# mackelab/poisson-gpfa

Hardware: AMD Instinct MI355X
Metric: EM iterations/sec (higher is better)
Workload: dtype f64

## Files before the change

poisson-gpfa_amd/csrc/core.hip:

```cpp
#include "ctx.h"
#include "model.h"
#include "dual.h"

using namespace pgpfa;

thread_local std::string g_err;
thread_local unsigned long long g_fail_count = 0;

int fail(const char* fmt, ...) {
  char buf[1024];
  va_list ap;
  va_start(ap, fmt);
  vsnprintf(buf, sizeof(buf), fmt, ap);
  va_end(ap);
  g_err = buf;
  ++g_fail_count;
  return 1;
}

int ensure_hbuf(pgpfa_ctx* c, size_t len) {
  if (len <= c->hbuf_len) return 0;
  if (c->hbuf) hipHostFree(c->hbuf);
  c->hbuf = nullptr;
  HIPC(hipHostMalloc((void**)&c->hbuf, len * sizeof(double)));
// ... 606 lines not shown
    hipLaunchKernelGGL((rbf_pivchol2_kernel<256, 4>), dim3(p), dim3(1024), pivchol2_lds(T, rmax, 1024, 4), st, c->Flr, Tp, T, c->tau, c->bin, c->eps, c->lr_tol, rmax,
                       c->d_rank);
  else if (T > 256)
    hipLaunchKernelGGL((rbf_pivchol_kernel<512, 2>), dim3(p), dim3(1024), shm, st, c->Flr, Tp, T, c->tau, c->bin, c->eps, c->lr_tol, rmax, c->d_rank);
  else
    hipLaunchKernelGGL((rbf_pivchol_kernel<256, 1>), dim3(p), dim3(256), shm, st, c->Flr, Tp, T, c->tau, c->bin, c->eps, c->lr_tol, rmax, c->d_rank);
  HIPC(hipGetLastError());
  return 0;
}

int build_lowrank(pgpfa_ctx* c, bool pivchol_launched) {
  const int p = c->p, T = c->T, Tp = c->Tp;
  if (pivchol_launched) HIPC(hipStreamWaitEvent(c->st, c->ev_join, 0));
  else CHK(launch_pivchol(c, c->st));
  std::vector<int> r(p);
  CHK(dl_enqueue(c, r.data(), c->d_rank, sizeof(int) * p));
  CHK(dl_flush(c));
  const bool thin_all = c->thin_products >= 2 && c->mfma && T >= 4;
  const int G = ((c->rank_gran == 4 || c->rank_gran == 8) && thin_all) ? c->rank_gran : 16;
  c->rk.assign(p, 0);
  c->roff.assign(p + 1, 0);
  c->rr.assign(p, 0);
  c->roff16.assign(p + 1, 0);
  int extent = 0;
  for (int k = 0; k < p; ++k) {
    c->rr[k] = round_up(std::max(r[k], 1), G);
    c->rk[k] = round_up(c->rr[k], 16);
    c->roff[k + 1] = c->roff[k] + c->rr[k];
    c->roff16[k + 1] = c->roff16[k] + c->rk[k];
    extent = std::max(extent, c->roff[k] + c->rk[k]);
  }
  c->rtot = c->roff[p];
  c->rtot16 = c->roff16[p];
  c->rank_compact = (G != 16);
  c->rpad = round_up(std::max(c->rtot, extent), NB);
  const int nblk = round_up(c->rtot16, NB) / 16;
  std::vector<int> lat(nblk, -1), col(nblk, 0);
  for (int k = 0; k < p; ++k)
    for (int b = c->roff16[k] / 16; b < c->roff16[k + 1] / 16; ++b) { lat[b] = k; col[b] = b * 16 - c->roff16[k]; }
  CHK(upload_list(c, c->d_blk_lat, lat));
  CHK(upload_list(c, c->d_blk_col, col));
  CHK(upload_list(c, c->d_roff, c->roff));
  CHK(upload_list(c, c->d_roff16, c->roff16));
  if (c->rank_compact) {
    const int n16 = round_up(c->rtot16, NB);
    std::vector<int> cmap(n16, -1), pmap(round_up(c->rtot, 16) + 16, 0);
    for (int k = 0; k < p; ++k)
      for (int j = 0; j < c->rr[k]; ++j) { cmap[c->roff16[k] + j] = c->roff[k] + j; pmap[c->roff[k] + j] = c->roff16[k] + j; }
    std::vector<int> nrtab((round_up(c->rtot, 16)) / 16, 0);
    for (size_t b = 0; b < nrtab.size(); ++b) {
      const int last = std::min((int)b * 16 + 15, c->rtot - 1);
      nrtab[b] = std::min(c->rtot16, round_up(pmap[last] + 1, 16));
    }
    CHK(upload_list(c, c->d_cmap, cmap));
    CHK(upload_list(c, c->d_nrtab, nrtab));
  }
  {
    std::vector<int> tft, tf;
    c->kr_ft_len = 0; c->kr_f_len = 0;
    for (int k = 0; k < p; ++k) {
      const int kb = (k * T) / 16 * 16, ke = std::min(c->npad, round_up((k + 1) * T, 16));
      for (int r0 = c->roff[k]; r0 < c->roff[k + 1]; r0 += 64) { tft.push_back(r0); tft.push_back(c->roff[k + 1]); tft.push_back(kb); tft.push_back(ke); }
      c->kr_ft_len = std::max(c->kr_ft_len, ke - kb);
      for (int i0 = k * T; i0 < (k + 1) * T; i0 += 64) { tf.push_back(i0); tf.push_back((k + 1) * T); tf.push_back(c->roff[k]); tf.push_back(c->roff[k + 1]); }
      c->kr_f_len = std::max(c->kr_f_len, c->rk[k]);
    }
    c->ntab_ft = (int)tft.size() / 4; c->ntab_f = (int)tf.size() / 4;
    if (tft.size() > c->tab_cap || tf.size() > c->tab_cap) return fail("internal: row-tile table overflow");
    CHK(upload_list(c, c->d_kr_ft, tft));
    CHK(upload_list(c, c->d_kr_f, tf));
    std::vector<int> hft, hf;
    for (int k = 0; k < p; ++k) {
      const int ngr = (c->rr[k] + 63) / 64, per = round_up((c->rr[k] + ngr - 1) / ngr, 4);
      for (int m0 = 0; m0 < c->rr[k]; m0 += per) { hft.push_back(k); hft.push_back(m0); hft.push_back(std::min(per, c->rr[k] - m0)); hft.push_back(c->roff[k]); }
      for (int t0 = 0; t0 < T; t0 += 256) { hf.push_back(k); hf.push_back(t0); hf.push_back(c->rk[k]); hf.push_back(c->roff[k]); }
    }
    std::vector<int> hs;
    for (int m0 = 0; m0 < c->rtot; m0 += 64) { hs.push_back(0); hs.push_back(m0); hs.push_back(std::min(64, c->rtot - m0)); hs.push_back(0); }
    c->nthin_s = (int)hs.size() / 4;
    if (hs.size() > c->tab_cap) return fail("internal: thin-product table overflow");
    CHK(upload_list(c, c->d_thin_s, hs));
    c->nthin_ft = (int)hft.size() / 4; c->nthin_f = (int)hf.size() / 4;
    if (hft.size() > c->tab_cap || hf.size() > c->tab_cap) return fail("internal: thin-product table overflow");
    CHK(upload_list(c, c->d_thin_ft, hft));
    CHK(upload_list(c, c->d_thin_f, hf));
  }
  if ((size_t)c->rpad <= (size_t)c->ld) {
    HIPC(hipMemsetAsync(c->Fbig, 0, (size_t)c->ld * c->rpad * sizeof(double), c->st));
    HIPC(hipMemsetAsync(c->FTbig, 0, (size_t)c->rpad * c->ld * sizeof(double), c->st));
    int rkmax = 0;
    for (int k = 0; k < p; ++k) rkmax = std::max(rkmax, c->rk[k]);
    hipLaunchKernelGGL(build_fbig_kernel, dim3(rkmax, p), dim3(128), 0, c->st, c->Flr, Tp, T, c->d_roff, c->Fbig, c->ld, c->FTbig, c->rpad);
    HIPC(hipGetLastError());
  }
  c->info["lowrank_rtot"] = c->rtot;
  c->info["lowrank_rtot16"] = c->rtot16;
  c->info["lowrank_compact"] = c->rank_compact ? 1.0 : 0.0;
  c->flr32_valid = false;
  return 0;
}


int resolve_trials(pgpfa_ctx* c, int n, const int32_t* idx, Trials* out, bool distinct) {
  if (idx == nullptr) {
    out->v.resize(c->R);
    for (int i = 0; i < c->R; ++i) out->v[i] = i;
// ... 35 lines not shown
  int ndev = 0;
  hipError_t e = hipGetDeviceCount(&ndev);
  if (e != hipSuccess || ndev < 1) return fail("no HIP device available (%s)", hipGetErrorString(e));
  if (device < 0 || device >= ndev) return fail("device %d out of range (%d devices)", device, ndev);
  HIPC(hipSetDevice(device));
  pgpfa_ctx* c = new pgpfa_ctx();
  c->device = device; c->q = q; c->p = p; c->T = T; c->R = R; c->bin = bin_ms;
  c->n = p * T;
  c->npad = round_up(c->n, NB);
  c->ld = c->npad;
  c->Tp = round_up(T, NB);
  hipError_t se = hipStreamCreateWithFlags(&c->st, hipStreamNonBlocking);
  if (se != hipSuccess) { delete c; return fail("hipStreamCreate: %s", hipGetErrorString(se)); }
  if (hipStreamCreateWithFlags(&c->st2, hipStreamNonBlocking) != hipSuccess || hipEventCreateWithFlags(&c->ev_fork, hipEventDisableTiming) != hipSuccess ||
      hipEventCreateWithFlags(&c->ev_join, hipEventDisableTiming) != hipSuccess) {
    (void)hipGetLastError();
    if (c->st2) { hipStreamDestroy(c->st2); c->st2 = nullptr; }
  }
  int rc = 0;
  const size_t slab = (size_t)c->Tp * c->Tp;
  rc |= dmalloc(c, &c->Y, (size_t)R * q * T);
  rc |= dmalloc(c, &c->C, (size_t)q * p); rc |= dmalloc(c, &c->d, q); rc |= dmalloc(c, &c->tau, p);
  rc |= dmalloc(c, &c->Kpad, slab * p); rc |= dmalloc(c, &c->Kinv, slab * p);
  rc |= dmalloc(c, &c->Xmode, (size_t)R * c->n + 64, true);
  rc |= dmalloc(c, &c->Xprev, (size_t)R * c->n + 64, true);
  c->mode_serial.assign(R, -10); c->prev_serial.assign(R, -10);
  rc |= dmalloc(c, &c->vsm, (size_t)R * T * p * p + 2048, true);
  rc |= dmalloc(c, &c->Pauto, slab * p, true);
  rc |= dmalloc(c, &c->Pacc, slab * p, true);
  c->gemm_part_len = (size_t)16 << 20;
  rc |= dmalloc(c, &c->gemm_part, c->gemm_part_len);
  c->qpad = round_up(q, 16);
  c->ccu_cols = round_up(p * (p + 1) / 2, 16);
  if (p <= 16) {
    dispatch_pw(p, [&](auto pw) { constexpr int PW = decltype(pw)::value; c->ccu_cols = round_up(PW * (PW + 1) / 2, 16); });
    rc |= dmalloc(c, &c->CCu, (size_t)c->qpad * c->ccu_cols + 64, true);
    rc |= dmalloc(c, &c->C16, (size_t)c->qpad * 16 + 64, true);
  }
  c->dual_npd = round_up(p * (p + 1) / 2, 16);
  c->dual_ncol = c->dual_npd + round_up(p, 16);
  rc |= dmalloc(c, &c->dual_tbl, (size_t)round_up(q, 128) * c->dual_ncol + 4096, true);
  rc |= dmalloc(c, &c->ppart, (size_t)p * (PACC_SPLITS + 1) * T * T + 256);
  c->vsmgp_ok.assign(R, 0);
  c->trial_snap.assign(R, -1);
  c->trial_dual.assign(R, 0);
  c->lam_resident.assign(R, 0);
  c->lam_valid.assign(R, 0);
  rc |= dmalloc(c, &c->Flr, slab * p + 256 * (size_t)c->Tp, true);
  rc |= dmalloc(c, &c->d_rank, p); rc |= dmalloc(c, &c->d_roff, p + 1); rc |= dmalloc(c, &c->d_roff16, p + 1);
  rc |= dmalloc(c, &c->d_cmap, (size_t)p * c->Tp + 2 * NB + 64); rc |= dmalloc(c, &c->d_nrtab, (size_t)p * c->Tp / 16 + 64);
  c->tab_cap = 4 * ((size_t)c->ld / 64 + 2 * (size_t)p + 4);
  rc |= dmalloc(c, &c->d_kr_ft, c->tab_cap); rc |= dmalloc(c, &c->d_kr_f, c->tab_cap);
  rc |= dmalloc(c, &c->sink, 128, true);
  rc |= dmalloc(c, &c->d_thin_ft, c->tab_cap); rc |= dmalloc(c, &c->d_thin_f, c->tab_cap); rc |= dmalloc(c, &c->d_thin_s, c->tab_cap);
  rc |= dmalloc(c, &c->Fbig, (size_t)c->ld * c->ld + 256 * (size_t)c->ld, true); rc |= dmalloc(c, &c->FTbig, (size_t)c->ld * c->ld + 256 * (size_t)c->ld, true);
  rc |= dmalloc(c, &c->Gbar, (size_t)T * p * p + 64); rc |= dmalloc(c, &c->Wtbar, (size_t)T * p * p + 64); rc |= dmalloc(c, &c->d_blk_lat, (size_t)p * c->Tp / 16 + 64); rc |= dmalloc(c, &c->d_blk_col, (size_t)p * c->Tp / 16 + 64);
  rc |= dmalloc(c, &c->vec, (size_t)q * (p + 1));
  rc |= dmalloc(c, &c->cdpart, (size_t)1024 * (p + 2) * q);
  rc |= dmalloc(c, &c->cdout, (size_t)(p + 2) * q + 8);
  rc |= dmalloc(c, &c->cdym, (size_t)(p + 1) * q + 8);
  rc |= dmalloc(c, &c->cdym_part, (size_t)1024 * (p + 1) * q);
  rc |= dmalloc(c, &c->last_trials, R);
  {
    const size_t NH = 1 + (size_t)(p + 1) + (size_t)(p + 1) * (p + 2) / 2;
    rc |= dmalloc(c, &c->cdhpart, (size_t)128 * NH * q);
    rc |= dmalloc(c, &c->cdhout, NH * q + 8);
    rc |= dmalloc(c, &c->cdcenter, (size_t)q * (p + 1));
    rc |= dmalloc(c, &c->cdpack, (size_t)q * (p + 3) + 8);
  }
  if (hipHostMalloc((void**)&c->h_pcg, 4 * sizeof(int), hipHostMallocMapped) != hipSuccess ||
      hipHostGetDevicePointer((void**)&c->d_hpcg, c->h_pcg, 0) != hipSuccess) { (void)hipGetLastError(); c->h_pcg = nullptr; c->d_hpcg = nullptr; }
  rc |= alloc_cholws(c, &c->kws, p * TAU_MULTI_MAX, c->Tp, true);
  c->kws.nact = round_up(T, 64);
  {
    const size_t nqmax = (size_t)p * TAU_MULTI_MAX;
    rc |= dmalloc(c, &c->tK, slab * nqmax); rc |= dmalloc(c, &c->tM, slab * nqmax); rc |= dmalloc(c, &c->tA1, slab * nqmax);
    rc |= dmalloc(c, &c->tA2, slab * nqmax);
    rc |= dmalloc(c, &c->tscal, 16 + 8 * nqmax); rc |= dmalloc(c, &c->tpart, 1024 + 64 * nqmax);
  }
  if (rc) { pgpfa_destroy(c); return 1; }
  e = hipStreamSynchronize(c->st);
  if (e != hipSuccess) { pgpfa_destroy(c); return fail("sync: %s", hipGetErrorString(e)); }
  if (const char* g = std::getenv("PGPFA_RANK_GRAN")) { const int v = std::atoi(g); if (v == 4 || v == 8 || v == 16) c->rank_gran = v; }
  c->info["n_pad"] = c->npad;
  c->info["counts_two_bytes"] = 0.0;
  c->info["arena_bytes"] = 0.0;
  c->info["last_eps_wt_norm"] = 0.0;
  c->info["last_eps_wt_rms"] = 0.0;
  c->info["last_split_cov"] = 0.0;
  c->info["last_yt_mix_fused"] = 0.0;
  for (const char* k : {"plan_ms_total", "plans", "set_params_calls", "last_retry_ms", "last_dense_retries", "last_param_step", "last_param_step_prev",
                        "last_fallback_no_descent", "last_fallback_line_search", "last_fallback_outer_cap", "arena_grow_ms_total", "last_cold_restarts"}) c->info[k] = 0.0;
  *out = c;
  return 0;
}

int pgpfa_destroy(pgpfa_ctx* c) {
  if (!c) return 0;
  hipSetDevice(c->device);
  if (c->st) hipStreamSynchronize(c->st);
  if (c->comm) ncclCommDestroy(c->comm);
  for (void* p : c->allocs) hipFree(p);
  if (c->vsmgp) hipFree(c->vsmgp);
  if (c->Flr32) hipFree(c->Flr32);
  if (c->lam_keep) hipFree(c->lam_keep);
  if (c->split_buf) hipFree(c->split_buf);
  if (c->Yhi) hipFree(c->Yhi);
  arena_release(c);
  if (c->hbuf) hipHostFree(c->hbuf);
  if (c->dl_stage) hipHostFree(c->dl_stage);
  if (c->hibuf) hipHostFree(c->hibuf);
  if (c->ring) hipHostFree(c->ring);
  if (c->h_pcg) hipHostFree(c->h_pcg);
  if (c->h_seq) hipHostFree(c->h_seq);
  for (auto e : c->prof.pool) hipEventDestroy(e);
  if (c->st2) { hipStreamSynchronize(c->st2); hipStreamDestroy(c->st2); }
  if (c->tau_pin) hipHostFree(c->tau_pin);
  if (c->ev_tau_fork) hipEventDestroy(c->ev_tau_fork);
  if (c->ev_tau_done) hipEventDestroy(c->ev_tau_done);
  if (c->ev_fork) hipEventDestroy(c->ev_fork);
  if (c->ev_join) hipEventDestroy(c->ev_join);
  if (c->st) hipStreamDestroy(c->st);
  delete c;
  return 0;
}

int pgpfa_set_option(pgpfa_ctx* c, const char* key, double v) {
  if (!c || !key) return fail("null argument");
  const std::string k(key);
  if (k == "newton_xtol") c->xtol = v;
  else if (k == "newton_max_iter") c->max_iter = (int)v;
  else if (k == "use_mfma") {
    const bool was = c->mfma;
    c->mfma = (v != 0.0);
    if (c->have_params && c->rank_gran != 16 && was != c->mfma)
      CHK(pgpfa_set_params(c, std::vector<double>(c->hC).data(), std::vector<double>(c->hd).data(), std::vector<double>(c->htau).data()));
  }
  else if (k == "cd_mfma") c->cd_mfma = (v != 0.0);
  else if (k == "cd_hess_mfma") c->cd_hess_mfma = (v != 0.0);
  else if (k == "cross_kernel") c->cross_kernel = (v != 0.0);
  else if (k == "cd_debug") c->cd_debug = (int)v;
  else if (k == "pcg_fused") c->pcg_fused = (int)v;
  else if (k == "pcg_w32") c->pcg_w32 = (v != 0.0);
  else if (k == "pcg_form") c->pcg_form = (int)v;
  else if (k == "pcg_vec32") c->pcg_vec32 = (int)v;
  else if (k == "pcg_rx32") c->pcg_rx32 = (int)v;
  else if (k == "pcg_adapt") c->pcg_adapt = (int)v;
  else if (k == "pcg_xcd") c->pcg_xcd = (int)v;
  else if (k == "mt_fill") c->mt_fill = (int)v;
  else if (k == "overlap_factors") c->overlap_factors = (int)v;
  else if (k == "mix_slot") c->mix_slot = (int)v;
  else if (k == "yt_mix") c->yt_mix = (v != 0.0);
  else if (k == "pivchol_pairs") c->pivchol_pairs = (v != 0.0);
  else if (k == "vsm_b4") c->vsm_b4 = (int)v;
  else if (k == "poisson_tiles") c->poisson_tiles = (int)v;
  else if (k == "yt_mix_dbg") c->yt_mix_dbg = (int)v;
  else if (k == "syrk_dbg") c->syrk_dbg = (int)v;
  else if (k == "syrk_tile") c->syrk_tile = (int)v;
  else if (k == "mix_wide") c->mix_wide = (int)v;
  else if (k == "thin_products") {
    const bool was = c->thin_products >= 2;
    c->thin_products = (int)v;
    if (c->have_params && c->rank_gran != 16 && was != (c->thin_products >= 2))
      CHK(pgpfa_set_params(c, std::vector<double>(c->hC).data(), std::vector<double>(c->hd).data(), std::vector<double>(c->htau).data()));
  }
  else if (k == "copy_kernels") c->copy_kernels = (v != 0.0);
  else if (k == "chord") c->chord = (v != 0.0);
  else if (k == "shared_pcg") c->shared_pcg = (v != 0.0);
  else if (k == "time_newton") c->time_newton = (v != 0.0);
  else if (k == "pcg_trace") c->pcg_trace = (v != 0.0);
  else if (k == "measure_mix") { c->measure_mix = (v != 0.0); c->info["last_eps_wt_norm"] = 0.0; c->info["last_eps_wt_rms"] = 0.0; }
  else if (k == "pcg_retire") c->pcg_retire = (v != 0.0);
  else if (k == "split_cov") c->split_cov = (v != 0.0);
  else if (k == "split_max_norm") c->split_max_norm = v;
  else if (k == "cov_mode") c->cov_mode = (int)v;
  else if (k == "lowrank_tol") {
    const bool changed = c->lr_tol != v;
    c->lr_tol = v;
    if (c->have_params && changed)
      CHK(pgpfa_set_params(c, std::vector<double>(c->hC).data(), std::vector<double>(c->hd).data(), std::vector<double>(c->htau).data()));
  }
  else if (k == "keep_trial_vsmgp") c->keep_trial_vsmgp = (v != 0.0);
  else if (k == "dual_lowrank") c->dual_lowrank = (v != 0.0);
  else if (k == "dual_f32") c->dual_f32 = (int)v;
  else if (k == "slab_row_align") c->slab_row_align = (v != 0.0);
  else if (k == "vsm_mfma") c->vsm_mfma = (v != 0.0);
  else if (k == "dual_gemm") c->dual_gemm = (v != 0.0);
  else if (k == "extrapolate_start") c->extrapolate = (v != 0.0);
  else if (k == "extrapolate_beta") c->extrapolate_beta = v;
  else if (k == "extrapolate_guard") c->extrapolate_guard = v;
  else if (k == "start_guard") c->start_guard = (v != 0.0);
  else if (k == "shared_min") c->shared_min = (int)v;
  else if (k == "pcg_inner") c->pcg_inner_max = std::max(1, (int)v);
  else if (k == "pcg_eta0") c->pcg_eta0 = v;
  else if (k == "splitk_target") c->splitk_target = std::max(1, (int)v);
  else if (k == "small_tile_below") c->small_tile_below = (int)v;
  else if (k == "f32_tile64") c->f32_tile64 = (int)v;
  else if (k == "splitk_below64") c->splitk_below64 = (int)v;
  else if (k == "pcg_outer_max") c->pcg_outer_max = (int)v;
  else if (k == "chord_xtol") c->chord_xtol = v;
  else if (k == "chord_rho") c->chord_rho = v;
  else if (k == "chord_max_step") c->chord_max_step = v;
  else if (k == "chord_max") c->chord_max = (int)v;
  else if (k == "chunk_trials") { if (c->B > 0) return fail("chunk_trials must be set before the first E-step"); c->chunk_opt = (int)v; }
  else if (k == "workspace_headroom") c->arena_headroom = std::max(1.0, v);
  else if (k == "rank_gran") { if (v != 4.0 && v != 8.0 && v != 16.0) return fail("rank_gran is 4, 8 or 16"); c->rank_gran = (int)v; if (c->have_params) CHK(pgpfa_set_params(c, std::vector<double>(c->hC).data(), std::vector<double>(c->hd).data(), std::vector<double>(c->htau).data())); }
  else if (k == "workspace_pool") { if (c->arena_cap > 0) return fail("workspace_pool must be set before the first E-step"); c->use_pool = (v != 0.0); }
  else if (k == "workspace_grow_budget_ms") c->grow_budget_ms = v;
  else if (k == "workspace_grow_floor_slots") c->grow_floor_slots = std::max(1, (int)v);
// ... 312 lines not shown
```

poisson-gpfa_amd/csrc/cov.hip:

```cpp
#include "ctx.h"
#include "model.h"
#include "split.h"
#include "ytmix.h"

using namespace pgpfa;

template <typename TIN>
void launch_post_vsm(pgpfa_ctx* c, const TIN* Mt, long long sM, int ncol, int ns, int full_range, const int* roff = nullptr, int ts = 0) {
  const int T = c->T, p = c->p;
  if (ts <= 0) ts = T;
  if (p > 10 && c->vsm_mfma) {
    const int CB = post_vsm_mfma_cb(p, sizeof(TIN) == 4);
    if (p <= 20 && c->vsm_b4) {
      constexpr int VW = 16 / (int)sizeof(TIN);
      const bool vec = c->vsm_b4 >= 2 && T % VW == 0 && ts % VW == 0 && c->ld % VW == 0 && sM % VW == 0 && (((size_t)Mt) & 15) == 0;
      auto go = [&](auto nbk, auto vv) {
        constexpr int NBK = decltype(nbk)::value;
        constexpr bool VEC = decltype(vv)::value;
        const size_t lds4 = (size_t)CB * post_vsm_b4_cs(p, VEC) * sizeof(TIN);
        constexpr int BINS = VEC ? 64 : 32;
        (void)hipFuncSetAttribute(reinterpret_cast<const void*>(&post_vsm_b4_kernel<NBK, TIN, VEC>), hipFuncAttributeMaxDynamicSharedMemorySize, (int)lds4);
        hipLaunchKernelGGL((post_vsm_b4_kernel<NBK, TIN, VEC>), dim3((T + BINS - 1) / BINS, ns), dim3(512), lds4, c->st, Mt, sM, c->ld, ncol, T, p, c->vsm,
                           c->ident, c->trial_of_slot, full_range, CB, roff, (int)GBN, ts);
      };
// ... 74 lines not shown
      g.M = T; g.N = T; g.K = c->npad - kal; g.alpha = 1.0; g.beta = 0.0;
      g.slots = c->ident; g.nbatch = nb; g.mode = GEMM_LOWER; g.kflags = KF_BEGIN_MAXRC;
      CHK(gemm(c, false, g));
      hipLaunchKernelGGL(scatter_vsmgp_kernel, dim3((unsigned)(((size_t)T * T + 255) / 256), nb), dim3(256), 0, c->st, c->ws.H, c->ws.sH, c->vsmgp,
                         T, p, k, c->trial_of_slot);
    }
  }
  prof_begin(c, TAG_VSM, (double)nb * c->npad * c->npad * p);
  launch_post_vsm(c, (const double*)c->ws.Mt, (long long)c->ws.sM, c->npad, nb, 0);
  prof_end(c);
  HIPC(hipGetLastError());
  return 0;
}


static int accumulate_split(pgpfa_ctx* c, const CholWS& lw, int nb, int ract, int Ts, bool skip_zero_cols, int ctile, bool fused) {
  const int T = c->T, p = c->p, Tp = c->Tp, rpad = c->rpad;
  const long long sW = (long long)T * p * p;
  const size_t tt = (size_t)T * T;
  (void)skip_zero_cols;
  constexpr int NS = 256, NG = PACC_SPLITS + 1;
  const size_t tq = (size_t)round_up(T, 16) * round_up(T, 16);
  if (!c->split_buf) {
    const size_t len = ((size_t)NS + NG + 3) * tq + 2 * (size_t)p * tt + 1024;
    if (hipMalloc((void**)&c->split_buf, len * sizeof(double)) != hipSuccess) { (void)hipGetLastError(); c->split_buf = nullptr; return fail("out of device memory for the split accumulation (%zu bytes)", len * sizeof(double)); }
    c->bytes += len * sizeof(double);
  }
  double* Spart = c->split_buf;
  double* Xpart = Spart + (size_t)NS * tq;
  double* Ssum = Xpart + (size_t)NG * tq;
  double* Xsum = Ssum + tq;
  double* Zb = Xsum + tq;
  double* T1 = Zb + tq;
  double* Xfull = T1 + (size_t)p * tt;
  float* D = reinterpret_cast<float*>(lw.H + (size_t)c->ld * rpad);
  const long long sD = 2 * (long long)lw.sH;
  const int ldd = c->ld;
  double mix_cols = 0.0;
  for (int k = 0; k < p; ++k) mix_cols += std::max(0, ract - (ctile > 0 ? (c->roff[k] / ctile) * ctile : 0));
  if (fused) {
    prof_begin(c, TAG_MIX, (double)nb * T * ((double)ract * ract + 16.0 * ract + (double)ract * (2.0 * p * p + p * (p + 1.0))));
    dispatch_pw(p, [&](auto pw) {
      constexpr int PW = decltype(pw)::value;
      if constexpr (PW <= 10) {
        YtMixArgs a{};
        a.F = c->Flr; a.Tp = Tp; a.Mts = lw.Mt; a.sM = (long long)lw.sM; a.rpad = rpad;
        a.D = D; a.sD = sD; a.ldd = ldd; a.G = c->Gbin; a.sG = sW;
        a.T = T; a.p = p; a.ract = ract; a.nbx = (T + YTM_BINS - 1) / YTM_BINS; a.nslots = nb; a.eps = c->eps;
        a.vsm = c->vsm; a.slots = c->ident; a.trial_of_slot = c->trial_of_slot; a.ts = Ts; a.dbg = c->yt_mix_dbg;
        a.roff = c->rank_compact ? c->d_roff16 : c->d_roff; a.cmap = c->rank_compact ? c->d_cmap : nullptr; a.nrtab = c->rank_compact ? c->d_nrtab : nullptr;
        a.ncmap = c->rank_compact ? round_up(c->rtot16, (int)NB) : 0;
        if (ytmix_lds(PW) + (size_t)a.ncmap * sizeof(int) > (size_t)160 * 1024) a.ncmap = 0;
        const size_t lds = ytmix_lds(PW) + (size_t)a.ncmap * sizeof(int);
        (void)hipFuncSetAttribute(reinterpret_cast<const void*>(&yt_mix_kernel<PW>), hipFuncAttributeMaxDynamicSharedMemorySize, (int)lds);
        hipLaunchKernelGGL(yt_mix_kernel<PW>, dim3((unsigned)(a.nbx * nb)), dim3(YTM_THREADS), lds, c->st, a);
      }
    });
    prof_end(c);
  } else {
  prof_begin(c, TAG_MIX, (double)nb * T * (mix_cols * 8.0 + (double)p * ract * 4.0));
  if (p > 16)
    hipLaunchKernelGGL((mix_vsm_wide2_kernel<20, true>), dim3((T + 63) / 64, nb), dim3(256), 0, c->st, lw.H, (long long)lw.sH, c->ld, c->Gbin, sW, T, p, ract, c->eps,
                       c->vsm, c->ident, c->trial_of_slot, Ts, c->sink, D, sD, ldd);
  else
  dispatch_pw(p, [&](auto pw) {
    constexpr int PW = decltype(pw)::value;
    if constexpr (PW <= 10) {
      if (c->mix_slot >= 3 && p == PW && ract % 4 == 0) {
        (void)hipFuncSetAttribute(reinterpret_cast<const void*>(&mix_slot3_kernel<PW, 128, 2>), hipFuncAttributeMaxDynamicSharedMemorySize, (int)mix_slot_lds(PW, 128));
        hipLaunchKernelGGL((mix_slot3_kernel<PW, 128, 2>), dim3((T + 127) / 128, nb), dim3(256), mix_slot_lds(PW, 128), c->st, (const double*)lw.H, (long long)lw.sH, c->ld, D, sD, ldd,
                           c->Gbin, sW, T, ract, c->eps, c->vsm, c->ident, c->trial_of_slot, c->d_roff, ctile, Ts);
        return;
      }
      if (c->mix_slot >= 2 && p == PW && ract % 4 == 0) {
        (void)hipFuncSetAttribute(reinterpret_cast<const void*>(&mix_slot2_kernel<PW, 256, 2>), hipFuncAttributeMaxDynamicSharedMemorySize, (int)mix_slot_lds(PW, 256));
        hipLaunchKernelGGL((mix_slot2_kernel<PW, 256, 2>), dim3((T + 255) / 256, nb), dim3(256), mix_slot_lds(PW, 256), c->st, (const double*)lw.H, (long long)lw.sH, c->ld, D, sD, ldd,
                           c->Gbin, sW, T, ract, c->eps, c->vsm, c->ident, c->trial_of_slot, c->d_roff, ctile, Ts);
        return;
      }
      if (c->mix_slot) {
        (void)hipFuncSetAttribute(reinterpret_cast<const void*>(&mix_slot_kernel<PW, 256, 2>), hipFuncAttributeMaxDynamicSharedMemorySize, (int)mix_slot_lds(PW, 256));
        hipLaunchKernelGGL((mix_slot_kernel<PW, 256, 2>), dim3((T + 255) / 256, nb), dim3(256), mix_slot_lds(PW, 256), c->st, (const double*)lw.H, (long long)lw.sH, c->ld, D, sD, ldd,
                           c->Gbin, sW, T, p, ract, c->eps, c->vsm, c->ident, c->trial_of_slot, c->d_roff, ctile, Ts);
        return;
      }
    }
    if constexpr (PW <= 16)
      hipLaunchKernelGGL(mix_vsm_split_kernel<PW>, dim3((T + 63) / 64, nb), dim3(256), 0, c->st, (const double*)lw.H, (long long)lw.sH, c->ld, D, sD, ldd,
                         c->Gbin, sW, T, p, ract, c->eps, c->vsm, c->ident, c->trial_of_slot, c->d_roff, ctile, Ts);
  });
  prof_end(c);
  }
  const int sps = std::max(1, (nb + PACC_SPLITS - 1) / PACC_SPLITS);
  const int ngroups = (nb + sps - 1) / sps;
  {
    SyrkF16Args a{};
    a.D = D; a.sD = sD; a.ldd = ldd; a.ts = Ts; a.part = c->ppart;
    a.T = T; a.p = p; a.ract = ract; a.nslots = nb; a.sps = sps; a.ngroups = ngroups;
    a.dbg = c->syrk_dbg;
    const int t256 = (T + 255) / 256;
    const bool big = c->syrk_tile >= 256 && T > 256 && (Ts & 3) == 0 && (ldd & 3) == 0 && t256 * 256 <= Ts && (((size_t)D) & 15) == 0 && (sD & 3) == 0;
    a.tiles = big ? t256 : (T + 127) / 128; a.ntiles = a.tiles * (a.tiles + 1) / 2;
    const long long blocks = (long long)a.ntiles * ngroups * p;
    prof_begin(c, TAG_VSM, 3.0 * (double)nb * ract * T * T * p);
    if (big) {
      const size_t lds = (size_t)4 * 2 * 256 * 32 * sizeof(_Float16);
      (void)hipFuncSetAttribute(reinterpret_cast<const void*>(&syrk256_f16x2_kernel), hipFuncAttributeMaxDynamicSharedMemorySize, (int)lds);
      hipLaunchKernelGGL(syrk256_f16x2_kernel, dim3((unsigned)blocks), dim3(512), lds, c->st, a);
// ... 466 lines not shown
```

poisson-gpfa_amd/csrc/ctx.h:

```cpp
#pragma once
#include <hip/hip_runtime.h>
#include <rccl/rccl.h>

#include <algorithm>
#include <limits>
#include <chrono>
#include <cmath>
#include <cstdarg>
#include <cstdio>
#include <cstring>
#include <deque>
#include <functional>
#include <map>
#include <string>
#include <type_traits>
#include <vector>

#include <mutex>
#include <rocprofiler-sdk-roctx/roctx.h>
#include "../../include/pgpfa.h"
#include "types.h"

using namespace pgpfa;

// ... 126 lines not shown
  double* dual_scr = nullptr; long long dual_sscr = 0;
  CholWS sws{};
  double *sU = nullptr, *sDinvT = nullptr, *Wbar = nullptr;
  double *Rv = nullptr, *Zv = nullptr, *Pv = nullptr, *Qv = nullptr;
  PcgCtl* pcgctl = nullptr;
  int* live = nullptr; float *pcg_ratio = nullptr, *pcg_eta = nullptr;
  int* live1 = nullptr;
  int* pcg_blk = nullptr;
  const int* cur_ndev = nullptr;
  bool live_gemm_collect = false;
  std::vector<std::pair<std::string, double>> live_gemms;
  bool pcg_retire = true;
  int* h_pcg = nullptr; int* d_hpcg = nullptr;
  float* W32 = nullptr;
  double* sc_part2 = nullptr;
  int pcg_fused = 1; bool pcg_w32 = true;
  int mt_fill = 1;
  int pcg_xcd = 1;
  int pcg_adapt = 1;
  int pcg_form = 2;
  int pcg_rx32 = 1;
  int pcg_vec32 = 1;
  double *Sv = nullptr, *cg_scal = nullptr;
  double *GbT = nullptr, *WbT = nullptr;
  double *sc_rz = nullptr, *sc_pq = nullptr, *sc_rr = nullptr, *sc_rr0 = nullptr, *sc_pack = nullptr;
  double* Flr = nullptr;
  double* Gbin = nullptr;
  int *d_rank = nullptr, *d_blk_lat = nullptr, *d_blk_col = nullptr, *d_roff = nullptr;
  int *d_kr_ft = nullptr, *d_kr_f = nullptr;
  int kr_ft_len = 0, kr_f_len = 0;
  int ntab_ft = 0, ntab_f = 0; size_t tab_cap = 0;
  int *d_thin_ft = nullptr, *d_thin_f = nullptr, *d_thin_s = nullptr;
  int nthin_ft = 0, nthin_f = 0, nthin_s = 0;
  int thin_products = 2;
  double *Fbig = nullptr, *FTbig = nullptr, *Gbar = nullptr, *Wtbar = nullptr;
  std::vector<int> rk, roff;
  std::vector<int> rr, roff16;
  int rtot = 0, rpad = 0, rtot16 = 0;
  int rank_gran = 4;
  bool rank_compact = false;
  int *d_roff16 = nullptr, *d_cmap = nullptr, *d_nrtab = nullptr;
  int cov_mode = 0;
  double lr_tol = 1e-10;
  bool plan_lowrank = false;
  size_t slab_elems = 0, mt_elems = 0, ws_mark = 0;
  char* arena = nullptr; size_t arena_cap = 0, arena_off = 0; int arena_mode = 0;
  int vmm = 0; size_t va_size = 0, vmm_gran = 0, vmm_granule = (size_t)1 << 30;
  std::vector<std::pair<hipMemGenericAllocationHandle_t, size_t>> vmm_chunks;
  double arena_headroom = 2.0;
  bool mt_dirty = false;
  bool last_cov_lowrank = false;
  bool shared_pcg = true;
  bool pcg_trace = false;
  double* sink = nullptr;
  int mix_wide = 1;
  int poisson_tiles = 2;
  int vsm_b4 = 2;
  int pivchol_pairs = 1;
  int yt_mix = 1;
  int syrk_tile = 256;
  int syrk_dbg = 0;
  int yt_mix_dbg = 0;
  int mix_slot = 3;
  bool cross_kernel = true;
  bool measure_mix = false;
  bool time_newton = false;
  int shared_min = 16, pcg_inner_min = 2, pcg_inner_max = 16, pcg_outer_max = 12;
  double pcg_eta0 = 1e-2;
  int splitk_target = 1280;
  int f32_tile64 = 1;
  int small_tile_below = 1 << 30;
  int splitk_below64 = 400;
  double *sc_f = nullptr, *sc_qxx = nullptr, *sc_qdx = nullptr, *sc_qdd = nullptr, *sc_dec = nullptr, *sc_smax = nullptr, *sc_alpha = nullptr;
  int *trial_of_slot = nullptr, *list_a = nullptr, *list_b = nullptr, *ident = nullptr;
  int* mask_of_slot = nullptr;
  bool mask_active = false;
  CholWS kws{};
  double *tK = nullptr, *tM = nullptr, *tA1 = nullptr, *tA2 = nullptr, *tscal = nullptr, *tpart = nullptr;
  double* hbuf = nullptr; size_t hbuf_len = 0;
  struct DlEntry { void* host; size_t off, bytes; };
  PcgCtl fused_ctl_host{};
  char* dl_stage = nullptr; size_t dl_used = 0; std::vector<DlEntry> dl_pending;
  char* dl_stage_dev = nullptr; char* ring_dev = nullptr;
  unsigned* h_seq = nullptr; unsigned* d_seq = nullptr; unsigned seq_next = 0;
  bool copy_kernels = true;
  unsigned long long dl_fail_mark = 0;
  int* hibuf = nullptr; size_t hibuf_len = 0;
  char* ring = nullptr; size_t ring_slot = 0; int ring_cur = 0, ring_pending = 0;
  std::map<std::string, double> info;
  std::vector<void*> allocs;
  size_t bytes = 0;
  Prof prof;
  ncclComm_t comm = nullptr;
  int rank = 0, nranks = 1;
  double* commbuf = nullptr; size_t commbuf_len = 0;
};

template <typename T>
int dmalloc(pgpfa_ctx* c, T** out, size_t count, bool zero = false) {
  void* p = nullptr;
  const size_t bytes = std::max<size_t>(count, 1) * sizeof(T);
  if (c->arena_mode) {
    const size_t aligned = (bytes + 255) & ~(size_t)255;
    *out = nullptr;
    if (c->arena_mode == 2) {
      if (c->arena_off + aligned > c->arena_cap) return fail("workspace arena overflow (%zu + %zu > %zu bytes)", c->arena_off, aligned, c->arena_cap);
      p = c->arena + c->arena_off;
      if (zero && hipMemsetAsync(p, 0, bytes, c->st) != hipSuccess) return fail("hipMemset failed");
      *out = reinterpret_cast<T*>(p);
    }
    c->arena_off += aligned;
    return 0;
  }
  hipError_t e = hipMalloc(&p, bytes);
// ... 127 lines not shown
```

poisson-gpfa_amd/csrc/ytmix.h:

```cpp
#pragma once
#include <hip/hip_runtime.h>

#include "split.h"

namespace pgpfa {

constexpr int YTM_KC = 256;
constexpr int YTM_AS = YTM_KC + 2;
constexpr int YTM_WAVES = 8;
constexpr int YTM_BINS = 16 * YTM_WAVES;
constexpr int YTM_THREADS = 64 * YTM_WAVES;

inline size_t ytmix_lds(int pw) { return ((size_t)(pw * (pw + 1) / 2) * YTM_BINS + 2 * 16 * (size_t)YTM_AS) * sizeof(double); }

struct YtMixArgs {
  const double* F; int Tp;
  const double* Mts; long long sM; int rpad;
  float* D; long long sD; int ldd;
  const double* G; long long sG;
  int T, p, ract, nbx, nslots; double eps;
  double* vsm;
  const int* slots; const int* trial_of_slot;
  const int* roff;
  const int* cmap; const int* nrtab;
  int ncmap;
  int ts;
  int dbg;
};

template <int PW>
__global__ __launch_bounds__(YTM_THREADS, 512 / YTM_THREADS) void yt_mix_kernel(YtMixArgs a) {
  typedef double v4d __attribute__((ext_vector_type(4)));
  typedef double v2d __attribute__((ext_vector_type(2)));
  constexpr int NPAIR = PW * (PW + 1) / 2;
  const int p = a.p, pp = p * p;
  extern __shared__ double ytm_lds[];
  double* Gs = ytm_lds;
  double* As = ytm_lds + NPAIR * YTM_BINS;
  const int tid = threadIdx.x, lane = tid & 63, l15 = lane & 15, l4 = lane >> 4;
  const int wave = __builtin_amdgcn_readfirstlane(tid >> 6);
  int w = blockIdx.x;
  const int total = gridDim.x;
  if ((total & 7) == 0) w = (w & 7) * (total >> 3) + (w >> 3);
  const int slot = a.slots[w / a.nbx];
  const int t0 = (w % a.nbx) * YTM_BINS;
  const int T = a.T;
  {
    const int bin = tid % YTM_BINS;
    const int part = __builtin_amdgcn_readfirstlane(tid / YTM_BINS);
    const int tb = t0 + bin < T ? t0 + bin : T - 1;
    const double* gsrc = a.G + (size_t)slot * a.sG + (size_t)tb * pp;
#pragma unroll
    for (int hi = 0; hi < PW; ++hi)
#pragma unroll
      for (int lo = 0; lo <= hi; ++lo) {
        const int idx = hi * (hi + 1) / 2 + lo;
        if ((idx & 3) == part) Gs[idx * YTM_BINS + bin] = hi < p ? gsrc[hi * p + lo] : 0.0;
      }
  }
  int ro[PW + 1];
#pragma unroll
  for (int k = 0; k <= PW; ++k) ro[k] = a.roff[k < p ? k : p];
  const int t = t0 + wave * 16 + l15;
  const int tc = t < T ? t : T - 1;
  const double* gl = Gs + wave * 16 + l15;
  const double* Ms = a.Mts + (size_t)slot * a.sM;
  const __amdgpu_buffer_rsrc_t d = wave_uniform_rsrc(a.D + (size_t)slot * a.sD, (size_t)a.ldd * a.ract * sizeof(float));
  const __amdgpu_buffer_rsrc_t fr = wave_uniform_rsrc(a.F, (size_t)p * a.Tp * a.Tp * sizeof(double));
  const unsigned flane = ((unsigned)l4 * (unsigned)a.Tp + (unsigned)tc) * 8u;
  const unsigned dlane = ((unsigned)l4 * (unsigned)a.ldd + (unsigned)tc) * 4u;
  double sums[NPAIR];
#pragma unroll
  for (int i = 0; i < NPAIR; ++i) sums[i] = 0.0;
  constexpr int TPC = YTM_THREADS / 16, NJ = YTM_KC / (2 * TPC);
  const int pcol = tid / TPC, prp = (tid % TPC) * 2;
  v2d tmp[NJ];
  int trow[NJ];
#pragma unroll
  for (int j = 0; j < NJ; ++j) { tmp[j] = v2d{0.0, 0.0}; trow[j] = 0; }
  int* const cmap_s = reinterpret_cast<int*>(As + 2 * 16 * YTM_AS);
  if (a.cmap)
    for (int e = tid; e < a.ncmap; e += YTM_THREADS) cmap_s[e] = a.cmap[e];
  const int* const cmap = a.cmap ? (a.ncmap > 0 ? cmap_s : a.cmap) : nullptr;
  if (a.cmap && a.ncmap > 0) __syncthreads();
  auto nr_of = [&](int b0) { return cmap ? a.nrtab[b0 >> 4] : b0 + 16; };
  auto panel_fetch = [&](int b0, int kc0, int kc1) {
    const double* src = Ms + (size_t)(b0 + pcol) * a.rpad;
#pragma unroll
    for (int j = 0; j < NJ; ++j) {
      const int i = kc0 + prp + 2 * TPC * j;
      tmp[j] = v2d{0.0, 0.0};
      trow[j] = -1;
      if (i < kc1 && !(a.dbg & 64)) {
        const int ic = cmap ? cmap[i] : i;
        trow[j] = ic;
        tmp[j] = *reinterpret_cast<const v2d*>(src + (ic < 0 ? 0 : ic));
      }
    }
  };
  auto panel_write = [&](int buf, int b0, int kc0, int kc1) {
    double* dst = As + (buf * 16 + pcol) * YTM_AS - kc0;
#pragma unroll
    for (int j = 0; j < NJ; ++j) {
      const int i = kc0 + prp + 2 * TPC * j;
      if (i < kc1) {
        v2d v = tmp[j];
        const int ic = trow[j];
        if (ic < 0 || ic > b0 + pcol) v.x = 0.0;
        if (ic < 0 || ic + 1 > b0 + pcol) v.y = 0.0;
        *reinterpret_cast<v2d*>(dst + i) = v;
      }
    }
  };
  const bool staged = !(a.dbg & 16);
  {
    const int nk0 = nr_of(0) < YTM_KC ? nr_of(0) : YTM_KC;
    if (staged) { panel_fetch(0, 0, nk0); panel_write(0, 0, 0, nk0); }
  }
  __syncthreads();
  int buf = 0;
  for (int b0 = 0; b0 < a.ract; b0 += 16) {
    const int nr = nr_of(b0);
    v4d acc[PW];
#pragma unroll
    for (int k = 0; k < PW; ++k) acc[k] = v4d{0.0, 0.0, 0.0, 0.0};
    auto frow_of = [&](int row) {
      int o = 0;
#pragma unroll
      for (int j = 1; j < PW; ++j) o = row >= ro[j] ? j * a.Tp - ro[j] : o;
      return o + row;
    };
    auto fetch4 = [&](int row, double& x0, double& x1, double& x2, double& x3) {
      const int fr0 = frow_of((row < nr && !(a.dbg & 1)) ? row : nr - 16);
      x0 = rsrc_load_f64(fr, flane, (unsigned)(fr0 * a.Tp) * 8u); x1 = rsrc_load_f64(fr, flane, (unsigned)((fr0 + 4) * a.Tp) * 8u);
      x2 = rsrc_load_f64(fr, flane, (unsigned)((fr0 + 8) * a.Tp) * 8u); x3 = rsrc_load_f64(fr, flane, (unsigned)((fr0 + 12) * a.Tp) * 8u);
    };
    double x0 = 0.0, x1 = 0.0, x2 = 0.0, x3 = 0.0, y0 = 0.0, y1 = 0.0, y2 = 0.0, y3 = 0.0;
    if (!(a.dbg & 2)) {
      const int fr0 = frow_of(0), fr1 = frow_of(16 < nr ? 16 : 0);
      x0 = rsrc_load_f64(fr, flane, (unsigned)(fr0 * a.Tp) * 8u); x1 = rsrc_load_f64(fr, flane, (unsigned)((fr0 + 4) * a.Tp) * 8u);
      x2 = rsrc_load_f64(fr, flane, (unsigned)((fr0 + 8) * a.Tp) * 8u); x3 = rsrc_load_f64(fr, flane, (unsigned)((fr0 + 12) * a.Tp) * 8u);
      y0 = rsrc_load_f64(fr, flane, (unsigned)(fr1 * a.Tp) * 8u); y1 = rsrc_load_f64(fr, flane, (unsigned)((fr1 + 4) * a.Tp) * 8u);
      y2 = rsrc_load_f64(fr, flane, (unsigned)((fr1 + 8) * a.Tp) * 8u); y3 = rsrc_load_f64(fr, flane, (unsigned)((fr1 + 12) * a.Tp) * 8u);
    }
    for (int kc0 = 0; kc0 < nr; kc0 += YTM_KC) {
      const int kc1 = kc0 + YTM_KC < nr ? kc0 + YTM_KC : nr;
      const double* arow = As + (buf * 16 + l15) * YTM_AS + l4 - kc0;
      if (!(a.dbg & 2))
#pragma unroll
      for (int k = 0; k < PW; ++k) {
        const int kb = ro[k] > kc0 ? ro[k] : kc0, ke = ro[k + 1] < kc1 ? ro[k + 1] : kc1;
        int i = kb;
        for (; i + 32 <= ke; i += 32) {
          const double* ar = arow + i;
          acc[k] = __builtin_amdgcn_mfma_f64_16x16x4f64(ar[0], x0, acc[k], 0, 0, 0);
          acc[k] = __builtin_amdgcn_mfma_f64_16x16x4f64(ar[4], x1, acc[k], 0, 0, 0);
          acc[k] = __builtin_amdgcn_mfma_f64_16x16x4f64(ar[8], x2, acc[k], 0, 0, 0);
          acc[k] = __builtin_amdgcn_mfma_f64_16x16x4f64(ar[12], x3, acc[k], 0, 0, 0);
          fetch4(i + 32, x0, x1, x2, x3);
          acc[k] = __builtin_amdgcn_mfma_f64_16x16x4f64(ar[16], y0, acc[k], 0, 0, 0);
          acc[k] = __builtin_amdgcn_mfma_f64_16x16x4f64(ar[20], y1, acc[k], 0, 0, 0);
          acc[k] = __builtin_amdgcn_mfma_f64_16x16x4f64(ar[24], y2, acc[k], 0, 0, 0);
          acc[k] = __builtin_amdgcn_mfma_f64_16x16x4f64(ar[28], y3, acc[k], 0, 0, 0);
          fetch4(i + 48, y0, y1, y2, y3);
        }
        if (i < ke) {
          const double* ar = arow + i;
          acc[k] = __builtin_amdgcn_mfma_f64_16x16x4f64(ar[0], x0, acc[k], 0, 0, 0);
          acc[k] = __builtin_amdgcn_mfma_f64_16x16x4f64(ar[4], x1, acc[k], 0, 0, 0);
          acc[k] = __builtin_amdgcn_mfma_f64_16x16x4f64(ar[8], x2, acc[k], 0, 0, 0);
          acc[k] = __builtin_amdgcn_mfma_f64_16x16x4f64(ar[12], x3, acc[k], 0, 0, 0);
          x0 = y0; x1 = y1; x2 = y2; x3 = y3;
          fetch4(i + 32, y0, y1, y2, y3);
        }
      }
      if (kc1 < nr) {
        const int nk1 = kc1 + YTM_KC < nr ? kc1 + YTM_KC : nr;
        if (staged) { panel_fetch(b0, kc1, nk1); panel_write(buf ^ 1, b0, kc1, nk1); if (!(a.dbg & 32)) __syncthreads(); }
        buf ^= 1;
      }
    }
    const int nb0 = b0 + 16;
    const bool more = staged && nb0 < a.ract;
    const int nrn = more ? nr_of(nb0) : 16;
    const int nk1 = nrn < YTM_KC ? nrn : YTM_KC;
#pragma unroll
    for (int r = 0; r < 4; r += 2) {
      double m[PW], n[PW];
#pragma unroll
      for (int k = 0; k < PW; ++k) { m[k] = 0.0; n[k] = 0.0; }
      if (!(a.dbg & 4))
#pragma unroll
      for (int hi = 0; hi < PW; ++hi)
#pragma unroll
        for (int lo = 0; lo <= hi; ++lo) {
          const double gg = gl[(hi * (hi + 1) / 2 + lo) * YTM_BINS];
          m[hi] += gg * acc[lo][r];
          n[hi] += gg * acc[lo][r + 1];
          if (lo != hi) { m[lo] += gg * acc[hi][r]; n[lo] += gg * acc[hi][r + 1]; }
        }
      if (t < T && !(a.dbg & 8)) {
#pragma unroll
        for (int k = 0; k < PW; ++k)
          if (k < p) {
            rsrc_store_f32(d, dlane, (unsigned)((b0 + 4 * r) * a.ldd + k * a.ts) * 4u, (float)(acc[k][r] - m[k]));
            rsrc_store_f32(d, dlane, (unsigned)((b0 + 4 * r + 4) * a.ldd + k * a.ts) * 4u, (float)(acc[k][r + 1] - n[k]));
          }
      }
#pragma unroll
      for (int hi = 0; hi < PW; ++hi)
#pragma unroll
        for (int lo = 0; lo <= hi; ++lo) sums[hi * (hi + 1) / 2 + lo] += m[hi] * m[lo];
#pragma unroll
      for (int hi = 0; hi < PW; ++hi)
#pragma unroll
        for (int lo = 0; lo <= hi; ++lo) sums[hi * (hi + 1) / 2 + lo] += n[hi] * n[lo];
      asm volatile("" ::: "memory");
    }
    if (more) { panel_fetch(nb0, 0, nk1); panel_write(buf ^ 1, nb0, 0, nk1); }
    if (staged && !(a.dbg & 32)) __syncthreads();
    buf ^= 1;
  }
#pragma unroll
  for (int i = 0; i < NPAIR; ++i) {
    sums[i] += __shfl_xor(sums[i], 16);
    sums[i] += __shfl_xor(sums[i], 32);
  }
  if (l4 != 0 || t >= T) return;
  double* vdst = a.vsm + ((size_t)a.trial_of_slot[slot] * T + t) * pp;
#pragma unroll
  for (int hi = 0; hi < PW; ++hi)
#pragma unroll
    for (int lo = 0; lo <= hi; ++lo) {
      if (hi >= p) continue;
      const double val = a.eps * gl[(hi * (hi + 1) / 2 + lo) * YTM_BINS] + sums[hi * (hi + 1) / 2 + lo];
      vdst[hi * p + lo] = val;
      vdst[lo * p + hi] = val;
    }
}

}
```

Before: 11.74.

## Stage yt_mix panels with direct global-to-LDS loads overlapped with MFMA

Adds a DMA variant of the yt_mix kernel that fills the shared-memory panel double buffer with global_load_lds_dwordx4, skipping the register round-trip. The next panel's load is issued before the current chunk's MFMA work and waited on afterwards, so staging overlaps compute. Padded rows read from a small zero buffer. A host-side check verifies that the compact rank map keeps rows in aligned pairs that can be copied as whole 16-byte units. The path is on by default and falls back to the old kernel when alignment preconditions fail. It relies on inline assembly that sets m0.

```diff
diff --git a/poisson-gpfa_amd/csrc/core.hip b/poisson-gpfa_amd/csrc/core.hip
--- a/poisson-gpfa_amd/csrc/core.hip
+++ b/poisson-gpfa_amd/csrc/core.hip
@@ -682,6 +682,9 @@
       const int last = std::min((int)b * 16 + 15, c->rtot - 1);
       nrtab[b] = std::min(c->rtot16, round_up(pmap[last] + 1, 16));
     }
+    for (int i = 0; i + 1 < n16; i += 2)
+      if (cmap[i] < 0 ? cmap[i + 1] >= 0 : ((cmap[i] & 1) != 0 || cmap[i + 1] != cmap[i] + 1))
+        return fail("rank tables: padded rows %d, %d map to slab rows %d, %d - not a pair the panel staging can move whole", i, i + 1, cmap[i], cmap[i + 1]);
     CHK(upload_list(c, c->d_cmap, cmap));
     CHK(upload_list(c, c->d_nrtab, nrtab));
   }
@@ -823,6 +826,7 @@
   c->tab_cap = 4 * ((size_t)c->ld / 64 + 2 * (size_t)p + 4);
   rc |= dmalloc(c, &c->d_kr_ft, c->tab_cap); rc |= dmalloc(c, &c->d_kr_f, c->tab_cap);
   rc |= dmalloc(c, &c->sink, 128, true);
+  rc |= dmalloc(c, &c->zero16, 2, true);
   rc |= dmalloc(c, &c->d_thin_ft, c->tab_cap); rc |= dmalloc(c, &c->d_thin_f, c->tab_cap); rc |= dmalloc(c, &c->d_thin_s, c->tab_cap);
   rc |= dmalloc(c, &c->Fbig, (size_t)c->ld * c->ld + 256 * (size_t)c->ld, true); rc |= dmalloc(c, &c->FTbig, (size_t)c->ld * c->ld + 256 * (size_t)c->ld, true);
   rc |= dmalloc(c, &c->Gbar, (size_t)T * p * p + 64); rc |= dmalloc(c, &c->Wtbar, (size_t)T * p * p + 64); rc |= dmalloc(c, &c->d_blk_lat, (size_t)p * c->Tp / 16 + 64); rc |= dmalloc(c, &c->d_blk_col, (size_t)p * c->Tp / 16 + 64);
@@ -926,6 +930,7 @@
   else if (k == "vsm_b4") c->vsm_b4 = (int)v;
   else if (k == "poisson_tiles") c->poisson_tiles = (int)v;
   else if (k == "yt_mix_dbg") c->yt_mix_dbg = (int)v;
+  else if (k == "yt_mix_dma") c->yt_mix_dma = (v != 0.0);
   else if (k == "syrk_dbg") c->syrk_dbg = (int)v;
   else if (k == "syrk_tile") c->syrk_tile = (int)v;
   else if (k == "mix_wide") c->mix_wide = (int)v;
diff --git a/poisson-gpfa_amd/csrc/cov.hip b/poisson-gpfa_amd/csrc/cov.hip
--- a/poisson-gpfa_amd/csrc/cov.hip
+++ b/poisson-gpfa_amd/csrc/cov.hip
@@ -150,8 +150,13 @@
         a.ncmap = c->rank_compact ? round_up(c->rtot16, (int)NB) : 0;
         if (ytmix_lds(PW) + (size_t)a.ncmap * sizeof(int) > (size_t)160 * 1024) a.ncmap = 0;
         const size_t lds = ytmix_lds(PW) + (size_t)a.ncmap * sizeof(int);
-        (void)hipFuncSetAttribute(reinterpret_cast<const void*>(&yt_mix_kernel<PW>), hipFuncAttributeMaxDynamicSharedMemorySize, (int)lds);
-        hipLaunchKernelGGL(yt_mix_kernel<PW>, dim3((unsigned)(a.nbx * nb)), dim3(YTM_THREADS), lds, c->st, a);
+        a.zero16 = c->zero16;
+        const bool dma = c->yt_mix_dma && c->zero16 && (!a.cmap || a.ncmap > 0) && rpad % 2 == 0 && lw.sM % 2 == 0 && (reinterpret_cast<uintptr_t>(lw.Mt) & 15) == 0;
+        auto launch = [&](auto kern) {
+          (void)hipFuncSetAttribute(reinterpret_cast<const void*>(kern), hipFuncAttributeMaxDynamicSharedMemorySize, (int)lds);
+          hipLaunchKernelGGL(kern, dim3((unsigned)(a.nbx * nb)), dim3(YTM_THREADS), lds, c->st, a);
+        };
+        if (dma) launch(&yt_mix_kernel<PW, true>); else launch(&yt_mix_kernel<PW, false>);
       }
     });
     prof_end(c);
diff --git a/poisson-gpfa_amd/csrc/ctx.h b/poisson-gpfa_amd/csrc/ctx.h
--- a/poisson-gpfa_amd/csrc/ctx.h
+++ b/poisson-gpfa_amd/csrc/ctx.h
@@ -202,6 +202,7 @@
   bool last_cov_lowrank = false;
   bool shared_pcg = true;
   bool pcg_trace = false;
+  double* zero16 = nullptr;
   double* sink = nullptr;
   int mix_wide = 1;
   int poisson_tiles = 2;
@@ -210,6 +211,7 @@
   int yt_mix = 1;
   int syrk_tile = 256;
   int syrk_dbg = 0;
+  int yt_mix_dma = 1;
   int yt_mix_dbg = 0;
   int mix_slot = 3;
   bool cross_kernel = true;
diff --git a/poisson-gpfa_amd/csrc/ytmix.h b/poisson-gpfa_amd/csrc/ytmix.h
--- a/poisson-gpfa_amd/csrc/ytmix.h
+++ b/poisson-gpfa_amd/csrc/ytmix.h
@@ -25,10 +25,18 @@
   const int* cmap; const int* nrtab;
   int ncmap;
   int ts;
+  const void* zero16;
   int dbg;
 };
 
-template <int PW>
+__device__ __forceinline__ void ytm_dma16(const void* gsrc, unsigned lds_dst) {
+  unsigned keep;
+  asm volatile("s_mov_b32 %0, m0\n\ts_mov_b32 m0, %2\n\ts_nop 0\n\tglobal_load_lds_dwordx4 %1, off\n\ts_mov_b32 m0, %0" : "=&s"(keep) : "v"(gsrc), "s"(lds_dst) : "memory");
+}
+template <int N>
+__device__ __forceinline__ void ytm_dma_wait() { asm volatile("s_waitcnt vmcnt(%0)" ::"n"(N) : "memory"); }
+
+template <int PW, bool DMA>
 __global__ __launch_bounds__(YTM_THREADS, 512 / YTM_THREADS) void yt_mix_kernel(YtMixArgs a) {
   typedef double v4d __attribute__((ext_vector_type(4)));
   typedef double v2d __attribute__((ext_vector_type(2)));
@@ -74,16 +82,18 @@
   for (int i = 0; i < NPAIR; ++i) sums[i] = 0.0;
   constexpr int TPC = YTM_THREADS / 16, NJ = YTM_KC / (2 * TPC);
   const int pcol = tid / TPC, prp = (tid % TPC) * 2;
-  v2d tmp[NJ];
-  int trow[NJ];
-#pragma unroll
-  for (int j = 0; j < NJ; ++j) { tmp[j] = v2d{0.0, 0.0}; trow[j] = 0; }
+  v2d tmp[DMA ? 1 : NJ];
+  int trow[DMA ? 1 : NJ];
+  if constexpr (!DMA) {
+#pragma unroll
+    for (int j = 0; j < NJ; ++j) { tmp[j] = v2d{0.0, 0.0}; trow[j] = 0; }
+  }
   int* const cmap_s = reinterpret_cast<int*>(As + 2 * 16 * YTM_AS);
   if (a.cmap)
     for (int e = tid; e < a.ncmap; e += YTM_THREADS) cmap_s[e] = a.cmap[e];
   const int* const cmap = a.cmap ? (a.ncmap > 0 ? cmap_s : a.cmap) : nullptr;
   if (a.cmap && a.ncmap > 0) __syncthreads();
-  auto nr_of = [&](int b0) { return cmap ? a.nrtab[b0 >> 4] : b0 + 16; };
+  auto nr_of = [&](int b0) { return cmap ? ((__attribute__((address_space(4))) const int*)a.nrtab)[b0 >> 4] : b0 + 16; };
   auto panel_fetch = [&](int b0, int kc0, int kc1) {
     const double* src = Ms + (size_t)(b0 + pcol) * a.rpad;
 #pragma unroll
@@ -112,10 +122,29 @@
       }
     }
   };
+  const unsigned as_lds = (unsigned)(unsigned long long)((__attribute__((address_space(3))) char*)As);
+  auto panel_dma = [&](int buf, int b0, int kc0, int kc1) {
+    const double* src0 = Ms + (size_t)(b0 + 2 * wave) * a.rpad;
+    int ic[2];
+    bool real[2];
+#pragma unroll
+    for (int h = 0; h < 2; ++h) {
+      const int i = kc0 + 128 * h + 2 * lane;
+      const bool in = i < kc1 && !(a.dbg & 64);
+      ic[h] = a.cmap ? ((__attribute__((address_space(3))) const int*)cmap_s)[in ? i : kc0] : i;
+      real[h] = in && ic[h] >= 0 && ic[h] < b0 + 16;
+    }
+#pragma unroll
+    for (int h = 0; h < 2; ++h)
+#pragma unroll
+      for (int c = 0; c < 2; ++c)
+        ytm_dma16(real[h] ? (const void*)(src0 + (size_t)c * a.rpad + ic[h]) : a.zero16, as_lds + (unsigned)((((buf * 16 + 2 * wave + c) * YTM_AS) + 128 * h) * sizeof(double)));
+  };
   const bool staged = !(a.dbg & 16);
   {
     const int nk0 = nr_of(0) < YTM_KC ? nr_of(0) : YTM_KC;
-    if (staged) { panel_fetch(0, 0, nk0); panel_write(0, 0, 0, nk0); }
+    if constexpr (DMA) { if (staged) panel_dma(0, 0, 0, nk0); ytm_dma_wait<0>(); }
+    else if (staged) { panel_fetch(0, 0, nk0); panel_write(0, 0, 0, nk0); }
   }
   __syncthreads();
   int buf = 0;
@@ -146,6 +175,12 @@
     for (int kc0 = 0; kc0 < nr; kc0 += YTM_KC) {
       const int kc1 = kc0 + YTM_KC < nr ? kc0 + YTM_KC : nr;
       const double* arow = As + (buf * 16 + l15) * YTM_AS + l4 - kc0;
+      if constexpr (DMA) {
+        if (staged) {
+          if (kc1 < nr) panel_dma(buf ^ 1, b0, kc1, kc1 + YTM_KC < nr ? kc1 + YTM_KC : nr);
+          else if (b0 + 16 < a.ract) panel_dma(buf ^ 1, b0 + 16, 0, nr_of(b0 + 16) < YTM_KC ? nr_of(b0 + 16) : YTM_KC);
+        }
+      }
       if (!(a.dbg & 2))
 #pragma unroll
       for (int k = 0; k < PW; ++k) {
@@ -176,7 +211,8 @@
       }
       if (kc1 < nr) {
         const int nk1 = kc1 + YTM_KC < nr ? kc1 + YTM_KC : nr;
-        if (staged) { panel_fetch(b0, kc1, nk1); panel_write(buf ^ 1, b0, kc1, nk1); if (!(a.dbg & 32)) __syncthreads(); }
+        if constexpr (DMA) { ytm_dma_wait<0>(); if (staged && !(a.dbg & 32)) __syncthreads(); }
+        else if (staged) { panel_fetch(b0, kc1, nk1); panel_write(buf ^ 1, b0, kc1, nk1); if (!(a.dbg & 32)) __syncthreads(); }
         buf ^= 1;
       }
     }
@@ -217,7 +253,8 @@
         for (int lo = 0; lo <= hi; ++lo) sums[hi * (hi + 1) / 2 + lo] += n[hi] * n[lo];
       asm volatile("" ::: "memory");
     }
-    if (more) { panel_fetch(nb0, 0, nk1); panel_write(buf ^ 1, nb0, 0, nk1); }
+    if constexpr (DMA) ytm_dma_wait<0>();
+    else if (more) { panel_fetch(nb0, 0, nk1); panel_write(buf ^ 1, nb0, 0, nk1); }
     if (staged && !(a.dbg & 32)) __syncthreads();
     buf ^= 1;
   }
```

Measured after the change: 12.44 (median of 6 runs). +6.0%, better.
